# lighttransport/nanort

Measured on AMD Instinct MI355X. Metric: Mrays/s (primary + 1-bounce) at 1920x1080, 1M-tri mesh; BVH build ms, higher is better.
Workload: dtype f32; 1 GPU; C3: Plane(1000,500) = 1,000,000 triangles fp32; 1920x1080 objrender-camera primaries + 1 cosine bounce per hit (2073600 + 2055142 rays per GPU per step); parallelism=replicated BVH, interleaved image rows per GPU

## Files before the change

### nanort_amd/csrc/api.hip

```cpp
#include <hip/hip_runtime.h>
#include <stdarg.h>
#include <stdio.h>
#include <stdlib.h>
#include <string.h>
#include <ctype.h>
#include <math.h>
#include <cmath>

#include <algorithm>
#include <atomic>
#include <chrono>
#include <mutex>
#include <thread>
#include <string>
#include <vector>

#include "kernels.h"
#include "launch_plan.h"
#ifdef NRT_PROF
#include "../../include/nanort_hip_prof.h"
#endif

using namespace nrt;

// ... 43 lines not shown

  struct LaunchSlot {
    uint32_t *d_cursor = nullptr;
    unsigned parity = 0;
    DevBuf spill, spill_tmin;
    DevBuf cyl_hits, cyl_bits;
    hipEvent_t done = nullptr;
    hipEvent_t t0 = nullptr, t1 = nullptr;
    hipStream_t stream = nullptr;
    bool used = false;
    DoneRec *h_done = nullptr, *d_done = nullptr;
    DoneCount *d_count = nullptr;
    uint32_t seq = 0;
    bool rec_pending = false;
    bool last_has_rec = false;
    bool last_timed = false;
  };
  static constexpr int kSlots = 4;
  LaunchSlot slots[kSlots];
  unsigned next_victim = 0;
  std::mutex launch_mutex;
  std::mutex host_mutex;
  unsigned long long *d_counters = nullptr;
  DevBuf st_rays, st_hits, st_mask;
  hipStream_t copy_in = nullptr, copy_out = nullptr;
  hipEvent_t ev_in[2] = {nullptr, nullptr}, ev_tr[2] = {nullptr, nullptr}, ev_out[2] = {nullptr, nullptr};
  int host_pipeline = 1;
  DevBuf b_wave_clock;
  uint32_t wave_clock_waves = 0;

  int lds_stack = kLdsStackDefault;
  unsigned chunk = 128, chunk_tail_pct = 0, refill_min = 44, trav_min = 16, leaf_min = 32;
  int f64_row_fetch = 1;
  unsigned trav_min4 = 24;
  unsigned num_parts = 8;
  unsigned debug_flags = 0;
  int subtree_rows = 1;
  int morton = 0;
  unsigned static_pct = 16;
  unsigned static_bands = 8;
  unsigned static_slice_groups = 2;
  unsigned max_blocks_per_cu = 0;
  int wide = 1, wide_stack = 10;
  int wide4 = 1;
  int wide4_big_ok = 1;
  int order4 = 0;
  int leaf_compact = 1;
  int dyn_head = 1;
  int wide_scramble = 0;
  struct { int lds_entries; unsigned blocks_per_cu; } occupancy[4][kNumPrimKinds] = {};

  hipEvent_t ev_b0 = nullptr, ev_b1 = nullptr;
  hipEvent_t ev_build_state = nullptr;
  void *build_state = nullptr;
  int last_timed_slot = -1;
  int launch_timing = 0;
  bool have_build_time = false;
  float segment_ms = 0.f;
  const char *last_kernel = "";
};

static nrt_status fail(nrt_ctx *c, nrt_status st, const char *fmt, ...) {
  char buf[512];
  va_list ap;
  va_start(ap, fmt);
  vsnprintf(buf, sizeof(buf), fmt, ap);
// ... 99 lines not shown

struct TunableDesc {
  const char *name;
  long long lo, hi;
  long long (*get)(const nrt_ctx *);
  void (*set)(nrt_ctx *, long long);
};
#define NRT_TUNABLE(name_, lo_, hi_, field_, type_)                                                          \
  {name_, lo_, hi_, [](const nrt_ctx *c) -> long long { return (long long)c->field_; },                      \
   [](nrt_ctx *c, long long v) { c->field_ = (type_)v; }}
static const TunableDesc kTunables[] = {
    NRT_TUNABLE("refill_min", 1, 64, refill_min, unsigned),
    NRT_TUNABLE("trav_min", 1, 64, trav_min, unsigned),
    NRT_TUNABLE("trav_min4", 1, 64, trav_min4, unsigned),
    NRT_TUNABLE("f64_row_fetch", 0, 1, f64_row_fetch, int),
    NRT_TUNABLE("leaf_min", 1, 64, leaf_min, unsigned),
    NRT_TUNABLE("chunk_tail_pct", 0, 100, chunk_tail_pct, unsigned),
    NRT_TUNABLE("parts", 1, kMaxParts, num_parts, unsigned),
    NRT_TUNABLE("static_pct", 0, 100, static_pct, unsigned),
    NRT_TUNABLE("static_bands", 1, 64, static_bands, unsigned),
    NRT_TUNABLE("static_slice_groups", 1, 64, static_slice_groups, unsigned),
    NRT_TUNABLE("blocks_per_cu", 0, 8, max_blocks_per_cu, unsigned),
    NRT_TUNABLE("debug", 0, 0x7FFFFFFF, debug_flags, unsigned),
    NRT_TUNABLE("morton", 0, 1, morton, int),
    NRT_TUNABLE("cyl_split", 1, 64, cyl_split, int),
    NRT_TUNABLE("cyl_seg_radii", 1, 1024, cyl_seg_radii, int),
#ifdef NRT_PROF
    NRT_TUNABLE("subtree_rows", 0, 1, subtree_rows, int),
#endif
    NRT_TUNABLE("wide", 0, 1, wide, int),
    NRT_TUNABLE("wide4_big", 0, 2, wide4_big_ok, int),
    NRT_TUNABLE("wide4", 0, 1, wide4, int),
    NRT_TUNABLE("leaf_compact", 0, 1, leaf_compact, int),
    NRT_TUNABLE("dyn_head", 0, 1, dyn_head, int),
    NRT_TUNABLE("order4", 0, 1, order4, int),
    NRT_TUNABLE("launch_timing", 0, 1, launch_timing, int),
    NRT_TUNABLE("host_pipeline", 0, 1, host_pipeline, int),
    NRT_TUNABLE("wide_scramble", 0, 1, wide_scramble, int),
    {"chunk", 32, 1 << 20, [](const nrt_ctx *c) -> long long { return c->chunk; },
     [](nrt_ctx *c, long long v) { c->chunk = (unsigned)(v / 32) * 32u; }},
    {"lds_stack", 16, 32, [](const nrt_ctx *c) -> long long { return c->lds_stack; },
     [](nrt_ctx *c, long long v) { if (v == 16 || v == 24 || v == 32) c->lds_stack = (int)v; }},
    {"wide_stack", 8, 16, [](const nrt_ctx *c) -> long long { return c->wide_stack; },
     [](nrt_ctx *c, long long v) { if (v == 8 || v == 10 || v == 12 || v == 16) c->wide_stack = (int)v; }},
};
#undef NRT_TUNABLE

static const TunableDesc *tunable_find(const char *name) {
  if (!name) return nullptr;
  for (const TunableDesc &d : kTunables)
    if (!strcmp(d.name, name)) return &d;
  return nullptr;
}
static bool tunable_set(nrt_ctx *c, const char *name, long long v) {
  const TunableDesc *d = tunable_find(name);
  if (!d) return false;
  d->set(c, std::min(d->hi, std::max(d->lo, v)));
  memset(c->occupancy, 0, sizeof(c->occupancy));
  return true;
}

extern "C" {

const char *nrtVersion(void) { return "libnanort_hip 0.1 (gfx950, HIP)"; }

nrt_status nrtHostAlloc(size_t bytes, void **out) {
// ... 783 lines not shown
  const bool profiled = (w.dbg & (32u | 8192u)) != 0u;
  a.nodes = (const typename Wire<T>::Node *)c->d_nodes;
  a.tris = (const LeafTri<T> *)c->d_tris;
  a.spheres = (const LeafSphere<T> *)c->d_tris;
  a.centers = (const T *)c->d_verts;
  a.cylinders = (const LeafCylinder<T> *)c->d_tris;
  a.cyl_test_cap = c->cyl_test_cap;
  a.curves = (const LeafCurve *)c->d_tris;
  a.curve_subdiv = c->curve_subdiv;
  a.wide = (const WideNode<T> *)c->d_wide;
  a.wide4 = w.wide4() ? (const Wide4Node<T> *)c->d_wide4 : nullptr;
  a.packed_leaves = c->packed_leaves;
  a.wide4_big = (w.wide4() && w.wide4_big) ? 1u : 0u;
  a.wide_below_4g = (c->f64_row_fetch && (uint64_t)c->num_branch_records * sizeof(WideNode<T>) < (1ull << 32)) ? 1u : 0u;
  a.root_is_branch = c->root_is_branch;
  a.debug_flags = w.dbg;
  a.range0 = l.opt->prim_ids_range[0];
  a.range1 = l.opt->prim_ids_range[1];
  a.skip_prim = l.opt->skip_prim_id;
  a.cull_back_face = l.opt->cull_back_face ? 1u : 0u;
  a.any_hit = l.kind == Query::Occlusion ? 1u : 0u;
  a.plain_options = w.plain_options ? 1u : 0u;
  a.root_test = c->tree_nested ? 0u : 1u;
  a.order4 = (c->order4 && w.wide4() && c->prim_kind == kPrimTriangles && l.kind != Query::Occlusion && !profiled) ? 1u : 0u;
  a.leaf_items = (c->leaf_compact && w.wide4() && c->prim_kind == kPrimTriangles && c->max_leaf_count <= 4u && !profiled) ? 1u : 0u;
  a.dyn_head = c->dyn_head ? 1u : 0u;
  a.counters = c->d_counters;
  a.wave_clock = (w.dbg & 8192u) ? (unsigned long long *)c->b_wave_clock.p : nullptr;
  a.chunk = c->chunk;
  a.chunk_tail_pct = c->chunk_tail_pct;
  a.refill_min = c->refill_min;
  a.trav_min = w.wide4() ? c->trav_min4 : c->trav_min;
  a.leaf_min = c->leaf_min;
}

template <typename T>
static void fill_launch_args(const TraverseLaunch<T> &l, const nrt_ctx::LaunchSlot *slot, const GridPlan &g, const DistributionPlan &d,
                             uint32_t levels, TraverseArgs<T> &a) {
  a.spill = (uint32_t *)slot->spill.p;
  a.spill_tmin = (T *)slot->spill_tmin.p;
  a.spill_stride = g.grid * kTraverseBlock;
  a.spill_levels = levels;
  a.ray_cursor = slot->d_cursor + (size_t)slot->parity * kCursorStrideWords * kMaxParts;
  a.next_cursor = slot->d_cursor + (size_t)(slot->parity ^ 1u) * kCursorStrideWords * kMaxParts;
  a.num_parts = g.parts;
  a.blocks_per_part = g.blocks_per_part;
  a.static_per_wave = d.static_per_wave;
  a.static_bands = d.static_bands;
  a.band_len = d.band_len;
  a.band_static = d.band_static;
  a.dyn_per_band = d.dyn_per_band;
  a.dyn_banded = d.dyn_banded;
  a.tail_begin = d.tail_begin;
  a.dyn_total = d.dyn_total;
  a.dyn_per_part = d.dyn_per_part;
  a.rays = l.rays;
  a.hits = l.hits;
  a.mask = l.mask;
  if (l.kind == Query::Cylinders || l.kind == Query::Curves) {
    a.hits = (typename Wire<T>::Hit *)slot->cyl_hits.p;
    a.mask = (uint8_t *)slot->cyl_bits.p;
  }
  a.num_rays = (uint32_t)l.n;
  a.num_batches = 1u;
  a.batch_anyhit = 0u;
  for (int k = 0; k < kMaxBatches; k++) {
// ... 57 lines not shown
  if (timed) {
    HIPCHK(c, hipEventRecord(slot->t1, s));
    slot->last_timed = true;
    c->last_timed_slot = (int)(slot - c->slots);
  }
  if (!use_rec) HIPCHK(c, hipEventRecord(slot->done, s));
  return NRT_OK;
}

template <typename T>
static nrt_status traverse_device(nrt_ctx *c, TraverseLaunch<T> l) {
  if (!l.opt) l.opt = &kDefaultTrace;
  std::lock_guard<std::mutex> lock(c->launch_mutex);
  nrt_status st = validate_launch(c, l);
  if (st || l.n == 0) return st;
  HIPCHK(c, hipSetDevice(c->device));
  HIPCHK(c, refit_stream_wait(c, l.stream));
  nrt_ctx::LaunchSlot *slot = nullptr;
  if ((st = take_slot(c, l.stream, &slot))) return st;
  const WalkChoice w = choose_walk(c, l);
  const GridPlan g = size_grid<T>(c, w, l.n);
  const uint32_t total_threads = g.grid * kTraverseBlock, total_waves = g.grid * (kTraverseBlock / kWave);
  const DistributionPlan d = plan_distribution((uint32_t)l.n, total_waves, g.parts, c->static_pct, c->static_bands, c->static_slice_groups, c->chunk);
  const uint32_t levels = plan_spill_levels(c->tree_depth, w.wide4(), (uint32_t)w.lds_entries);
  if (levels) {
    if ((st = ensure(c, slot->spill, (size_t)levels * total_threads * sizeof(uint32_t)))) return st;
    if (w.wide() && (st = ensure(c, slot->spill_tmin, (size_t)levels * total_threads * sizeof(T)))) return st;
  }
  if (l.kind == Query::Cylinders || l.kind == Query::Curves) {
    if ((st = ensure(c, slot->cyl_hits, (size_t)l.n * sizeof(typename Wire<T>::Hit)))) return st;
    if ((st = ensure(c, slot->cyl_bits, (size_t)l.n))) return st;
  }
  if (w.dbg & 8192u) {
    if ((st = ensure(c, c->b_wave_clock, (size_t)total_waves * 3 * sizeof(unsigned long long)))) return st;
    c->wave_clock_waves = total_waves;
  }
  TraverseArgs<T> a;
  fill_walk_args(c, l, w, a);
  fill_launch_args(l, slot, g, d, levels, a);
  return enqueue_launch(c, l, w, slot, a, g.grid);
}

const uint64_t kStagedRays = 1ull << 26;

template <typename T, typename MakeLaunch>
static nrt_status staged_host_loop(nrt_ctx *c, const typename Wire<T>::Ray *rays, uint64_t n, uint64_t chunk, size_t rec_bytes, size_t flag_bytes,
                                   void *recs, void *flags, MakeLaunch make) {
  const size_t ray_bytes = sizeof(typename Wire<T>::Ray);
  for (uint64_t off = 0; off < n; off += chunk) {
    const uint64_t m = std::min(chunk, n - off);
    nrt_status st;
    if ((st = ensure(c, c->st_rays, m * ray_bytes)) || (rec_bytes && (st = ensure(c, c->st_hits, m * rec_bytes))) || (st = ensure(c, c->st_mask, m * flag_bytes)))
      return st;
    HIPCHK(c, hipMemcpyAsync(c->st_rays.p, rays + off, m * ray_bytes, hipMemcpyHostToDevice, c->stream));
    if ((st = traverse_device<T>(c, make(m)))) return st;
    if (recs) HIPCHK(c, hipMemcpyAsync((char *)recs + off * rec_bytes, c->st_hits.p, m * rec_bytes, hipMemcpyDeviceToHost, c->stream));
    if (flags) HIPCHK(c, hipMemcpyAsync((char *)flags + off * flag_bytes, c->st_mask.p, m * flag_bytes, hipMemcpyDeviceToHost, c->stream));
    HIPCHK(c, hipStreamSynchronize(c->stream));
  }
  return NRT_OK;
}
static bool is_pinned_host(const void *p) {
  hipPointerAttribute_t at;
  if (hipPointerGetAttributes(&at, p) != hipSuccess) {
    (void)hipGetLastError();
    return false;
  }
// ... 542 lines not shown
    nrt_ctx::LaunchSlot &sl = c->slots[c->last_timed_slot];
    if (sl.last_has_rec) {
      if (wait_record(sl) != hipSuccess) return -1.f;
      const unsigned long long b = sl.h_done->t_begin, e = sl.h_done->t_end;
      const hipStream_t s = sl.stream;
      lock.unlock();
      if (hipStreamSynchronize(s) != hipSuccess) return -1.f;
      return e >= b ? (float)((double)(e - b) * 1e-5) : -1.f;
    }
    if (!sl.last_timed) return -1.f;
    t0 = sl.t0;
    t1 = sl.t1;
  }
  if (hipEventSynchronize(t1) != hipSuccess) return -1.f;
  float ms = -1.f;
  if (hipEventElapsedTime(&ms, t0, t1) != hipSuccess) return -1.f;
  return ms;
}

const char *nrtLastKernelName(const nrt_ctx *c) { return c ? c->last_kernel : ""; }

#ifdef NRT_PROF
int nrtDebugCounters(nrt_ctx *c, unsigned long long *out, int cap) {
  if (!c || !out || cap < 16) return 1;
  if (hipStreamSynchronize(c->stream) != hipSuccess) return 1;
  if (hipDeviceSynchronize() != hipSuccess) return 1;
  return hipMemcpy(out, c->d_counters, 16 * sizeof(unsigned long long), hipMemcpyDeviceToHost) == hipSuccess ? 0 : 1;
}

long nrtDebugWaveClocks(nrt_ctx *c, unsigned long long *out, long cap) {
  if (!c || !out || !c->b_wave_clock.p) return -1;
  if (hipDeviceSynchronize() != hipSuccess) return -1;
  const long n = std::min<long>(cap, (long)c->wave_clock_waves);
  if (hipMemcpy(out, c->b_wave_clock.p, (size_t)n * 3 * sizeof(unsigned long long), hipMemcpyDeviceToHost) != hipSuccess) return -1;
  return (long)c->wave_clock_waves;
}

#endif

float nrtLastBuildMs(nrt_ctx *c) {
  if (!c || !c->have_build_time) return -1.f;
  return c->stats.build_secs * 1e3f;
}

}
```

### nanort_amd/csrc/common.h

```cpp
#pragma once

#include <hip/hip_runtime.h>
#include <stddef.h>
#include <stdint.h>
#include <stdlib.h>

#include "../../include/nanort_hip.h"
#include "walk_variant.h"

#ifdef NRT_ROCTX
#include <rocprofiler-sdk-roctx/roctx.h>
namespace nrt {
struct RoctxRange {
  explicit RoctxRange(const char *msg) { roctxRangePushA(msg); }
  ~RoctxRange() { roctxRangePop(); }
};
}
#define NRT_RANGE_CAT2(a, b) a##b
#define NRT_RANGE_CAT(a, b) NRT_RANGE_CAT2(a, b)
#define NRT_RANGE(msg) ::nrt::RoctxRange NRT_RANGE_CAT(nrt_range_, __LINE__)(msg)
#define NRT_RANGE_PUSH(msg) roctxRangePushA(msg)
#define NRT_RANGE_POP() roctxRangePop()
#else
#define NRT_RANGE(msg) do { } while (0)
// ... 94 lines not shown
};
static_assert(sizeof(LeafCurve) == 64, "LeafCurve");

template <typename T>
struct alignas(16) WideNode {
  T box0[6];
  T box1[6];
  uint32_t c0, c1;
  int32_t axis;
  uint32_t pad;
};
template <>
struct alignas(16) WideNode<double> {
  double mn[3][2];
  double mx[3][2];
  uint32_t c0, c1;
  int32_t axis;
  uint32_t pad;
};
static_assert(sizeof(WideNode<float>) == 64, "WideNode<float>");
static_assert(sizeof(WideNode<double>) == 112, "WideNode<double>");
template <typename T>
struct alignas(16) Wide4Node {
  T bmin[3][4];
  T bmax[3][4];
  uint32_t c[4];
  int32_t axis0, axis1, axis2;
  uint32_t pad;
};
static_assert(sizeof(Wide4Node<float>) == 128, "Wide4Node<float>");
static_assert(sizeof(Wide4Node<double>) == 224, "Wide4Node<double>");
constexpr uint32_t kWide4Empty = 0xFFFFFFFFu;
constexpr uint32_t kLeafBit = 0x80000000u;
constexpr uint32_t kPackedFirstBits = 27;
constexpr uint32_t kPackedFirstMask = (1u << kPackedFirstBits) - 1u;
constexpr uint32_t kPackedMaxCount = 16;

struct TreeViewF32 {
  const nrt_node_f32 *nodes;
  const uint32_t *indices;
  const void *wide;
  const void *wide4;
  const void *prims;
  uint32_t num_nodes, num_indices;
  uint32_t packed_leaves, root_is_branch, tree_nested, prim_kind, tree_depth;
  uint32_t max_leaf_count;
  uint64_t generation;
};

struct SceneInst {
  const void *wide;
  const void *wide4;
  const void *tris;
  const nrt_node_f32 *nodes;
  uint32_t packed_leaves, root_is_branch, tree_nested, pad;
  float inv_xform[4][4];
  float inv_xform33[4][4];
  float xform[4][4];
  float xbmin[3], xbmax[3];
  uint32_t id, pad2;
};
static_assert(sizeof(SceneInst) == 272, "SceneInst");
__device__ __forceinline__ bool scene_node_interval(const nrt_ray_f32 &r, const float xbmin[3], const float xbmax[3], float &t_min_out) {
  float tmin = r.min_t, tmax = r.max_t;
  float tn[3], tf[3];
#pragma unroll
// ... 134 lines not shown
  BatchPtrs batches[kMaxBatches];
  uint32_t range0, range1, skip_prim;
  uint32_t cull_back_face;
  uint32_t any_hit;
  uint32_t plain_options;
  uint32_t root_test;
  uint32_t leaf_items;
  uint32_t order4;
  uint32_t *spill;
  T *spill_tmin;
  uint32_t spill_stride;
  uint32_t spill_levels;
  uint32_t *ray_cursor;
  uint32_t *next_cursor;
  uint32_t num_parts;
  uint32_t static_per_wave;
  uint32_t static_bands;
  uint32_t band_len;
  uint32_t band_static;
  uint32_t dyn_per_band;
  uint32_t dyn_banded;
  uint32_t tail_begin;
  uint32_t dyn_total;
  uint32_t dyn_per_part;
  uint32_t blocks_per_part;
  uint32_t dyn_head;
  unsigned long long *counters;
  unsigned long long *wave_clock;
  uint32_t chunk;
  uint32_t chunk_tail_pct;
  uint32_t refill_min;
  uint32_t trav_min;
  uint32_t leaf_min;
  DoneRec *done_rec;
  DoneCount *done_count;
  uint32_t done_seq;
  uint32_t done_publish;
  const LeafCurve *curves;
  uint32_t curve_subdiv;
};

}
```

### nanort_amd/csrc/traverse.hip

```cpp
#include "kernels.h"
#include "traverse_dev.h"

#include <algorithm>

namespace nrt {

template <typename A>
static void launch_persistent(const void *kernel, unsigned grid, const A &args, hipStream_t s) {
  void *params[] = {(void *)&args};
  (void)hipLaunchKernel(kernel, dim3(grid), dim3(kTraverseBlock), params, 0, s);
}
static int resident_blocks(const void *kernel, int fallback) {
  int n = 0;
  if (hipOccupancyMaxActiveBlocksPerMultiprocessor(&n, kernel, kTraverseBlock, 0) != hipSuccess || n < 1) n = fallback;
  return n > 8 ? 8 : n;
}

template <typename T, bool COUNT, int STACK>
__global__ __launch_bounds__(kTraverseBlock) void k_traverse(const TraverseArgs<T> a) {
  __shared__ uint32_t s_stack[STACK][kTraverseBlock];

  typedef typename Wire<T>::Node Node;
  typedef typename Wire<T>::Ray Ray;
  typedef typename Wire<T>::Hit Hit;
// ... 712 lines not shown
  T tt_i = T(0), uu_i = T(0), vv_i = T(0);
  if (ok) {
    const T Az = sz * Akz, Bz = sz * Bkz, Cz = sz * Ckz;
    const T D = U * Az + V * Bz + W * Cz;
    const T rcp = T(1.0) / det;
    tt_i = D * rcp;
    uu_i = V * rcp;
    vv_i = W * rcp;
  }
  const unsigned long long okm_ = __ballot(ok);
  bool got_ = false;
  uint32_t win_ = 0;
  for (uint32_t k2_ = 0; k2_ < kmax_; k2_++) {
    const uint32_t src_ = (base_ + k2_) & 63u;
    const T ttk = __int_as_float(__builtin_amdgcn_ds_bpermute((int)(src_ << 2), __float_as_int(tt_i)));
    const bool okk = (k2_ < cnt) & (((okm_ >> src_) & 1ull) != 0ull);
    const bool acc = okk & !(ttk > L.hit_t) & !(ttk < L.min_t);
    L.hit_t = acc ? ttk : L.hit_t;
    win_ = acc ? src_ : win_;
    got_ = got_ | acc;
  }
  if (__ballot(got_) != 0ull) {
    const int wa_ = (int)(win_ << 2);
    const T uw = __int_as_float(__builtin_amdgcn_ds_bpermute(wa_, __float_as_int(uu_i)));
    const T vw = __int_as_float(__builtin_amdgcn_ds_bpermute(wa_, __float_as_int(vv_i)));
    const uint32_t pw = (uint32_t)__builtin_amdgcn_ds_bpermute(wa_, (int)prim_i);
    L.u = got_ ? uw : L.u;
    L.v = got_ ? vw : L.v;
    L.prim = got_ ? pw : L.prim;
  }
  return true;
}

template <typename T, int STACK, bool STATS, int KIND, bool PLAIN = false, bool CLOCK = false, int WIDTH = 2, int ORDER = 0>
__global__ __launch_bounds__(kTraverseBlock, (WIDTH == 4 && sizeof(T) == 4) ? NRT_W4_WAVES : 1) void k_traverse_wide(const TraverseArgs<T> a) {
  static_assert(WIDTH == 2 || WIDTH == 4, "one or two tree levels per step");
  static_assert(KIND != kPrimCurves || sizeof(T) == 4, "curves are fp32 only, as their example");
  static_assert(ORDER == 0 || (WIDTH == 4 && sizeof(T) == 4), "distance order / leaf items are variants of the fp32 two-level step");
  static_assert((ORDER & 2) == 0 || (KIND == kPrimTriangles && !STATS), "leaf items: triangle records, production instantiations");
  static_assert((ORDER & 4) == 0 || ((ORDER & 1) == 0 && KIND == kPrimTriangles && !STATS && !CLOCK), "records addressed by 64-bit offsets: the default walk of triangle trees");
  constexpr bool LEAFC = (ORDER & 2) != 0;
  constexpr bool BIG = (ORDER & 4) != 0;
  typedef typename std::conditional<BIG, uint64_t, uint32_t>::type RecOff;
  __shared__ uint32_t s_item_owner[LEAFC ? kTraverseBlock / kWave : 1][LEAFC ? kWave : 1];
  __shared__ uint32_t s_item_rec[LEAFC ? kTraverseBlock / kWave : 1][LEAFC ? kWave : 1];
  typedef StackEntry<T> SE;
  __shared__ typename SE::type s_stack[STACK][kTraverseBlock];

  typedef typename Wire<T>::Node Node;
  typedef typename Wire<T>::Ray Ray;
  typedef typename Wire<T>::Hit Hit;

  const unsigned tid = threadIdx.x;
  const unsigned lane = lane_id();
  const unsigned gslot = blockIdx.x * kTraverseBlock + tid;
  const bool cull = a.cull_back_face != 0;

  NRT_BATCH_TABLE_SETUP();
  Lane<T> L;
  uint32_t rid = kInvalid;
  uint32_t cur = 0;
  int state = W_IDLE;
  int sp = 0;
  const bool clocked = CLOCK && a.wave_clock != nullptr;
  unsigned long long clk_begin = 0ull, clk_dry = 0ull;
  if (clocked) clk_begin = __builtin_amdgcn_s_memrealtime();
  Claim ck;
  claim_init<T>(a, ck);
  if (blockIdx.x == 0 && threadIdx.x < kMaxParts)
    __hip_atomic_store(a.next_cursor + kCursorStrideWords * threadIdx.x, 0u, __ATOMIC_RELAXED, __HIP_MEMORY_SCOPE_AGENT);
  done_begin<T>(a);
  unsigned long long st_it1 = 0, st_act1 = 0, st_idle2 = 0, st_it2 = 0, st_act2 = 0, st_refills = 0, st_refilled = 0, st_entries2 = 0;
  uint32_t st_steps = 0, st_tris = 0;
  unsigned long long st_t_refill = 0, st_t_p1 = 0, st_t_p2 = 0, st_act2b = 0, st_stamp = 0;
  unsigned long long st_it1_s = 0, st_act1_s = 0, st_it2_s = 0, st_act2_s = 0;

#define NRT_WRITE_RESULT()                              \
  do {                                                  \
    const bool hit_ = L.hit_t < L.max_t;                \
    Hit h_;                                             \
    h_.u = hit_ ? L.u : T(0);                           \
    h_.v = hit_ ? L.v : T(0);                           \
    if (STATS && (a.debug_flags & 64u)) {               \
      h_.u = T(st_steps);                               \
      h_.v = T(st_tris);                                \
    }                                                   \
    h_.t = hit_ ? L.hit_t : L.max_t;                    \
    h_.prim_id = hit_ ? L.prim : kInvalid;              \
    Hit *hp_ = a.hits;                                  \
    uint8_t *mp_ = a.mask;                              \
    if (multi) {                                        \
      const BatchPtrs bp_ = s_tbl[batch_of<T>(a, rid)]; \
      hp_ = (Hit *)bp_.hits_v;                          \
      mp_ = bp_.mask_v;                                 \
    }                                                   \
    if (hp_) store_hit_nt<T>(hp_ + rid, h_);            \
    if (mp_) mp_[rid] = hit_ ? (KIND == kPrimCylinders ? (uint8_t)(1u | (L.cap << 1)) : (uint8_t)1) : (uint8_t)0; \
  } while (0)

// ... 38 lines not shown
            rp_ = (const Ray *)s_tbl[b_].rays_v;
            bq_ = (a.batch_anyhit >> b_) & 1u;
          }
          const Ray r = (a.debug_flags & 4u) ? rp_[rid] : load_ray_nt<T>(rp_ + rid);
          lane_init<T>(L, r);
          L.pk |= bq_ << 9;
          sp = 0;
          if (STATS) st_steps = st_tris = 0;
          if (a.root_is_branch && !a.root_test) {
            cur = 0u;
            state = W_TRAV;
          } else if (a.root_is_branch) {
            const Node root = a.nodes[0];
            cur = 0u;
            state = slab_test<T>(L, root.bmin, root.bmax) ? W_TRAV : W_POP;
          } else {
            const Node root = a.nodes[0];
            const bool root_hit = slab_test<T>(L, root.bmin, root.bmax);
            cur = a.packed_leaves ? (((root.data[0] - 1u) << kPackedFirstBits) | root.data[1]) : 0u;
            state = root_hit ? W_LEAF : W_POP;
          }
          if (a.debug_flags & 2u) state = W_POP;
        }
        if (STATS) {
          st_refills++;
          st_refilled += take;
        }
        ck.next += take;
        fresh = __ballot(state == W_IDLE);
      }
      idle = __ballot(state == W_IDLE);
    }
    if (clocked && ck.exhausted && clk_dry == 0ull) clk_dry = __builtin_amdgcn_s_memrealtime();
    if (idle == ~0ull) {
      if (ck.exhausted) break;
      continue;
    }

    if (STATS) {
      const unsigned long long now_ = __builtin_amdgcn_s_memtime();
      st_t_refill += now_ - st_stamp;
      st_stamp = now_;
    }
    unsigned n_wait_leaf = (unsigned)__builtin_popcountll(__ballot(state == W_LEAF));
    while (state == W_TRAV || state == W_POP) {
      if (STATS) {
        st_it1++;
        st_act1 += (unsigned)__builtin_popcountll(__ballot(true));
        if (!ck.exhausted) {
          st_it1_s++;
          st_act1_s += (unsigned)__builtin_popcountll(__ballot(true));
        }
      }
#pragma unroll
      for (int u_ = 0; u_ < ((WIDTH == 4 && sizeof(T) == 4 && !STATS) ? NRT_W4_P1_UNROLL : ((WIDTH == 2 && sizeof(T) == 8 && !STATS) ? NRT_W2_F64_P1_UNROLL : 1)); u_++) {
      if (state == W_POP) NRT_POP_ENTRY();
      if (state == W_TRAV) {
        if (STATS) st_steps++;
        if constexpr (WIDTH == 4) {
#if NRT_W4_PRESEL
          if constexpr (sizeof(T) == 4) {
            const char *wb_ = reinterpret_cast<const char *>(a.wide4);
            const RecOff rec_ = (RecOff)cur << 7;
            const Slab4<float> sl = slab4_presel<RecOff>(L, wb_, rec_);
            const Wide4Tail w = *reinterpret_cast<const Wide4Tail *>(wb_ + (size_t)rec_ + 96);
            if constexpr ((ORDER & 1) == 1)
// ... 16 lines not shown
#endif
#if NRT_W2_F64_PRESEL
          bool stepped_ = false;
          if constexpr (sizeof(T) == 8) {
            if (a.wide_below_4g) {
              const char *wb_ = reinterpret_cast<const char *>(a.wide);
              const uint32_t rec_ = cur * (uint32_t)sizeof(WideNode<double>);
              const SlabPair<double> sl = slab_pair_presel(L, wb_, rec_);
              const WideTail w = *reinterpret_cast<const WideTail *>(wb_ + (size_t)rec_ + 96);
              NRT_STEP_NODE_SL(sl, w);
              stepped_ = true;
            }
          }
          if (!stepped_)
#endif
          {
          const WideNode<T> w = a.wide[cur];
#ifdef NRT_PROBE_EXTRA_VALU
          {
            float f_ = __uint_as_float(cur);
            for (int x_ = 0; x_ < NRT_PROBE_EXTRA_VALU; x_++) asm volatile("v_fma_f32 %0, %0, %0, %0" : "+v"(f_));
            asm volatile("" :: "v"(f_));
          }
#endif
          NRT_STEP_NODE(w);
          }
#ifdef NRT_PROBE_EXTRA_LOADS
          asm volatile("" :: "v"(d0_));
#endif
        }
      }
      }
      n_wait_leaf += (unsigned)__builtin_popcountll(__ballot(state == W_LEAF));
      if ((unsigned)__builtin_popcountll(__ballot(state == W_TRAV || state == W_POP)) < a.trav_min &&
          (n_wait_leaf != 0u || !ck.exhausted))
        break;
    }

    if (STATS) {
      const unsigned long long now_ = __builtin_amdgcn_s_memtime();
      st_t_p1 += now_ - st_stamp;
      st_stamp = now_;
    }
    const unsigned n_leaf = (unsigned)__builtin_popcountll(__ballot(state == W_LEAF));
    const bool refill_due = !ck.exhausted && (unsigned)__builtin_popcountll(__ballot(state == W_IDLE)) >= a.refill_min;
    if (n_leaf != 0u && !(n_leaf < a.leaf_min && refill_due)) {
      uint32_t cnt = 0, first = 0;
      if (state == W_LEAF) {
        if (a.packed_leaves) {
          cnt = (cur >> kPackedFirstBits) + 1u;
          first = cur & kPackedFirstMask;
        } else {
          const Node *nd = a.nodes + cur;
          cnt = nd->data[0];
          first = nd->data[1];
        }
      }
      if (a.debug_flags & 1u) cnt = 0;
      if (STATS) {
        st_entries2++;
        st_idle2 += (unsigned)__builtin_popcountll(__ballot(state == W_IDLE));
      }
      bool items_done_ = false;
      if constexpr (LEAFC) {
        items_done_ = leaf_items_one_trip<PLAIN, uint32_t>(L, cnt, a.tris, first, lane, s_item_owner[tid / kWave], s_item_rec[tid / kWave], a.range0, a.range1,
                                                 a.skip_prim, cull);
      }
      if (items_done_) {
      } else if constexpr (KIND == kPrimTriangles && (WIDTH == 4 ? NRT_W4_TRI_UNROLL : NRT_W2_TRI_UNROLL) > 1) {
// ... 15 lines not shown
#pragma unroll
          for (uint32_t j = 0; j < U_; j++) {
            if (PLAIN)
              tri_test<T, true>(L, t_[j], i + j < cnt, 0u, 0u, 0u, false);
            else
              tri_test<T>(L, t_[j], i + j < cnt, a.range0, a.range1, a.skip_prim, cull);
          }
        }
      } else if constexpr (!STATS && KIND == kPrimSpheres && NRT_SPHERE_UNROLL > 1) {
        for (uint32_t i = 0; __ballot(i < cnt) != 0ull; i += NRT_SPHERE_UNROLL) {
          LeafSphere<T> s_[NRT_SPHERE_UNROLL];
#pragma unroll
          for (uint32_t j = 0; j < NRT_SPHERE_UNROLL; j++) s_[j] = a.spheres[first + (i + j < cnt ? i + j : 0u)];
#pragma unroll
          for (uint32_t j = 0; j < NRT_SPHERE_UNROLL; j++) sphere_test<T>(L, s_[j], i + j < cnt, a.range0, a.range1);
        }
      } else
      for (uint32_t i = 0; __ballot(i < cnt) != 0ull; i++) {
        if (STATS) {
          st_it2++;
          st_act2 += (unsigned)__builtin_popcountll(__ballot(i < cnt));
          if (i < cnt) st_tris++;
        }
        NRT_TEST_PRIM(first + (i < cnt ? i : 0u), i < cnt);
      }
      if (a.any_hit | a.batch_anyhit) sp = (state == W_LEAF && L.hit_t < L.max_t && (a.any_hit != 0u || (L.pk & 512u) != 0u)) ? 0 : sp;
      state = (state == W_LEAF) ? W_POP : state;
    }
    if (STATS) st_t_p2 += __builtin_amdgcn_s_memtime() - st_stamp;
  }
  if (rid != kInvalid) NRT_WRITE_RESULT();
#undef NRT_WRITE_RESULT
#undef NRT_TEST_PRIM
  done_end<T>(a, lane);
  if (clocked && lane == 0u) {
    unsigned long long *rec = a.wave_clock + 3ull * (size_t)(gslot / kWave);
    const unsigned long long clk_end = __builtin_amdgcn_s_memrealtime();
    rec[0] = clk_begin;
    rec[1] = clk_dry == 0ull ? clk_end : clk_dry;
    rec[2] = clk_end;
  }
  if (STATS && lane == 0) {
    atomicAdd(&a.counters[0], st_it1);
    atomicAdd(&a.counters[1], st_act1);
    atomicAdd(&a.counters[2], st_idle2);
    atomicAdd(&a.counters[3], st_it2);
    atomicAdd(&a.counters[4], st_act2);
    atomicAdd(&a.counters[5], st_refills);
    atomicAdd(&a.counters[6], st_refilled);
    atomicAdd(&a.counters[7], st_entries2);
    atomicAdd(&a.counters[8], st_t_refill);
    atomicAdd(&a.counters[9], st_t_p1);
    atomicAdd(&a.counters[10], st_t_p2);
    atomicAdd(&a.counters[11], st_act2b);
    atomicAdd(&a.counters[12], st_it1_s);
    atomicAdd(&a.counters[13], st_act1_s);
    atomicAdd(&a.counters[14], st_it2_s);
    atomicAdd(&a.counters[15], st_act2_s);
  }
}

template <typename R>
__device__ __forceinline__ R load_global_record(const R *p) {
  R r;
  if constexpr (sizeof(R) % 16 == 0 && alignof(R) >= 16) {
    typedef uint32_t u4g __attribute__((ext_vector_type(4)));
    const u4g __attribute__((address_space(1))) *g = (const u4g __attribute__((address_space(1))) *)p;
    u4g *d = reinterpret_cast<u4g *>(&r);
#pragma unroll
    for (unsigned q = 0; q < sizeof(R) / 16; q++) d[q] = g[q];
  } else {
    static_assert(sizeof(R) % 4 == 0, "whole words");
    const uint32_t __attribute__((address_space(1))) *g = (const uint32_t __attribute__((address_space(1))) *)p;
// ... 981 lines not shown
```

Measured before the change: 6814 Mrays/s.

## Spread tail rays across lane quads for cooperative wide4 traversal

Once the ray pool is exhausted and a wave has at most tail_quad live rays, their state is compacted with ds_bpermute so each ray is owned by a 4-lane quad. The quad then processes one ray together: each lane tests one child box of a wide4 node, stack pushes are ordered through DPP quad reductions, and leaf triangles are split four ways with a quad-wide closest-hit vote. This targets the long low-occupancy tail of divergent waves, at the cost of a large extra code path that can add register pressure and shuffle overhead. It also adds wave-clock stamps for the 16/8/4-live points and grows the wave clock record to six words.

```diff
diff --git a/nanort_amd/csrc/api.hip b/nanort_amd/csrc/api.hip
--- a/nanort_amd/csrc/api.hip
+++ b/nanort_amd/csrc/api.hip
@@ -99,6 +99,7 @@
   int lds_stack = kLdsStackDefault;
   unsigned chunk = 128, chunk_tail_pct = 0, refill_min = 44, trav_min = 16, leaf_min = 32;
   int f64_row_fetch = 1;
+  unsigned tail_quad = 4;
   unsigned trav_min4 = 24;
   unsigned num_parts = 8;
   unsigned debug_flags = 0;
@@ -264,6 +265,7 @@
     NRT_TUNABLE("wide4_big", 0, 2, wide4_big_ok, int),
     NRT_TUNABLE("wide4", 0, 1, wide4, int),
     NRT_TUNABLE("leaf_compact", 0, 1, leaf_compact, int),
+    NRT_TUNABLE("tail_quad", 0, 16, tail_quad, unsigned),
     NRT_TUNABLE("dyn_head", 0, 1, dyn_head, int),
     NRT_TUNABLE("order4", 0, 1, order4, int),
     NRT_TUNABLE("launch_timing", 0, 1, launch_timing, int),
@@ -1113,6 +1115,7 @@
   a.refill_min = c->refill_min;
   a.trav_min = w.wide4() ? c->trav_min4 : c->trav_min;
   a.leaf_min = c->leaf_min;
+  a.tail_lanes = c->tail_quad;
 }
 
 template <typename T>
@@ -1236,7 +1239,7 @@
     if ((st = ensure(c, slot->cyl_bits, (size_t)l.n))) return st;
   }
   if (w.dbg & 8192u) {
-    if ((st = ensure(c, c->b_wave_clock, (size_t)total_waves * 3 * sizeof(unsigned long long)))) return st;
+    if ((st = ensure(c, c->b_wave_clock, (size_t)total_waves * kWaveClockWords * sizeof(unsigned long long)))) return st;
     c->wave_clock_waves = total_waves;
   }
   TraverseArgs<T> a;
@@ -1845,7 +1848,7 @@
   if (!c || !out || !c->b_wave_clock.p) return -1;
   if (hipDeviceSynchronize() != hipSuccess) return -1;
   const long n = std::min<long>(cap, (long)c->wave_clock_waves);
-  if (hipMemcpy(out, c->b_wave_clock.p, (size_t)n * 3 * sizeof(unsigned long long), hipMemcpyDeviceToHost) != hipSuccess) return -1;
+  if (hipMemcpy(out, c->b_wave_clock.p, (size_t)n * kWaveClockWords * sizeof(unsigned long long), hipMemcpyDeviceToHost) != hipSuccess) return -1;
   return (long)c->wave_clock_waves;
 }
 
diff --git a/nanort_amd/csrc/common.h b/nanort_amd/csrc/common.h
--- a/nanort_amd/csrc/common.h
+++ b/nanort_amd/csrc/common.h
@@ -150,6 +150,7 @@
 static_assert(sizeof(Wide4Node<double>) == 224, "Wide4Node<double>");
 constexpr uint32_t kWide4Empty = 0xFFFFFFFFu;
 constexpr uint32_t kLeafBit = 0x80000000u;
+constexpr int kWaveClockWords = 6;
 constexpr uint32_t kPackedFirstBits = 27;
 constexpr uint32_t kPackedFirstMask = (1u << kPackedFirstBits) - 1u;
 constexpr uint32_t kPackedMaxCount = 16;
@@ -350,6 +351,7 @@
   uint32_t refill_min;
   uint32_t trav_min;
   uint32_t leaf_min;
+  uint32_t tail_lanes;
   DoneRec *done_rec;
   DoneCount *done_count;
   uint32_t done_seq;
diff --git a/nanort_amd/csrc/traverse.hip b/nanort_amd/csrc/traverse.hip
--- a/nanort_amd/csrc/traverse.hip
+++ b/nanort_amd/csrc/traverse.hip
@@ -768,6 +768,16 @@
   return true;
 }
 
+__device__ __forceinline__ uint32_t quad_or(uint32_t x) {
+  x |= (uint32_t)__builtin_amdgcn_update_dpp(0, (int)x, 0xB1, 0xF, 0xF, true);
+  x |= (uint32_t)__builtin_amdgcn_update_dpp(0, (int)x, 0x4E, 0xF, 0xF, true);
+  return x;
+}
+template <int K>
+__device__ __forceinline__ float quad_bcast(float v) {
+  return __int_as_float(__builtin_amdgcn_update_dpp(0, __float_as_int(v), K * 0x55, 0xF, 0xF, true));
+}
+
 template <typename T, int STACK, bool STATS, int KIND, bool PLAIN = false, bool CLOCK = false, int WIDTH = 2, int ORDER = 0>
 __global__ __launch_bounds__(kTraverseBlock, (WIDTH == 4 && sizeof(T) == 4) ? NRT_W4_WAVES : 1) void k_traverse_wide(const TraverseArgs<T> a) {
   static_assert(WIDTH == 2 || WIDTH == 4, "one or two tree levels per step");
@@ -778,6 +788,7 @@
   constexpr bool LEAFC = (ORDER & 2) != 0;
   constexpr bool BIG = (ORDER & 4) != 0;
   typedef typename std::conditional<BIG, uint64_t, uint32_t>::type RecOff;
+  constexpr bool QUAD = WIDTH == 4 && sizeof(T) == 4 && KIND == kPrimTriangles && !STATS && (ORDER & 1) == 0 && !BIG;
   __shared__ uint32_t s_item_owner[LEAFC ? kTraverseBlock / kWave : 1][LEAFC ? kWave : 1];
   __shared__ uint32_t s_item_rec[LEAFC ? kTraverseBlock / kWave : 1][LEAFC ? kWave : 1];
   typedef StackEntry<T> SE;
@@ -800,7 +811,20 @@
   int sp = 0;
   const bool clocked = CLOCK && a.wave_clock != nullptr;
   unsigned long long clk_begin = 0ull, clk_dry = 0ull;
+  unsigned long long clk_l16 = 0ull, clk_l8 = 0ull, clk_l4 = 0ull;
   if (clocked) clk_begin = __builtin_amdgcn_s_memrealtime();
+#define NRT_TAIL_N (a.tail_lanes < 16u ? a.tail_lanes : 16u)
+#define NRT_CLOCK_LIVE(live_)                                                  \
+  do {                                                                         \
+    if constexpr (CLOCK) {                                                     \
+      if (clocked && ck.exhausted && clk_l4 == 0ull && (live_) <= 16u) {       \
+        const unsigned long long now_ = __builtin_amdgcn_s_memrealtime();      \
+        if (clk_l16 == 0ull) clk_l16 = now_;                                   \
+        if (clk_l8 == 0ull && (live_) <= 8u) clk_l8 = now_;                    \
+        if ((live_) <= 4u) clk_l4 = now_;                                      \
+      }                                                                        \
+    }                                                                          \
+  } while (0)
   Claim ck;
   claim_init<T>(a, ck);
   if (blockIdx.x == 0 && threadIdx.x < kMaxParts)
@@ -905,6 +929,213 @@
       idle = __ballot(state == W_IDLE);
     }
     if (clocked && ck.exhausted && clk_dry == 0ull) clk_dry = __builtin_amdgcn_s_memrealtime();
+    NRT_CLOCK_LIVE(64u - (unsigned)__builtin_popcountll(idle));
+    if constexpr (QUAD) {
+      const unsigned live_n_ = 64u - (unsigned)__builtin_popcountll(idle);
+      if (ck.exhausted && live_n_ != 0u && live_n_ <= NRT_TAIL_N) {
+        if (state == W_IDLE && rid != kInvalid) NRT_WRITE_RESULT();
+        const unsigned q_ = lane >> 2, j_ = lane & 3u;
+        uint32_t src_ = 0u;
+        {
+          unsigned k_ = 0u;
+          for (unsigned long long m_ = ~idle; m_ != 0ull; m_ &= m_ - 1ull, k_++) src_ = (q_ == k_) ? (uint32_t)__builtin_ctzll(m_) : src_;
+        }
+        const bool has_ = q_ < live_n_;
+        const int sa_ = (int)(src_ << 2);
+#define NRT_QMOVE_F(x_) x_ = __int_as_float(__builtin_amdgcn_ds_bpermute(sa_, __float_as_int(x_)))
+#define NRT_QMOVE_U(x_) x_ = (uint32_t)__builtin_amdgcn_ds_bpermute(sa_, (int)(x_))
+        NRT_QMOVE_F(L.org0);
+        NRT_QMOVE_F(L.org1);
+        NRT_QMOVE_F(L.org2);
+        NRT_QMOVE_F(L.inv0);
+        NRT_QMOVE_F(L.inv1);
+        NRT_QMOVE_F(L.inv2);
+        NRT_QMOVE_F(L.min_t);
+        NRT_QMOVE_F(L.max_t);
+        NRT_QMOVE_F(L.hit_t);
+        NRT_QMOVE_F(L.Sx);
+        NRT_QMOVE_F(L.Sy);
+        NRT_QMOVE_F(L.Sz);
+        NRT_QMOVE_F(L.u);
+        NRT_QMOVE_F(L.v);
+        NRT_QMOVE_U(L.pk);
+        NRT_QMOVE_U(L.prim);
+        NRT_QMOVE_U(rid);
+        NRT_QMOVE_U(cur);
+        state = __builtin_amdgcn_ds_bpermute(sa_, state);
+        sp = __builtin_amdgcn_ds_bpermute(sa_, sp);
+#undef NRT_QMOVE_F
+#undef NRT_QMOVE_U
+        L.so0 = (L.pk & 1u) ? 48u : 0u;
+        L.so1 = (L.pk & 2u) ? 48u : 0u;
+        L.so2 = (L.pk & 4u) ? 48u : 0u;
+        state = has_ ? state : W_IDLE;
+        rid = has_ ? rid : kInvalid;
+        sp = has_ ? sp : 0;
+        const unsigned otid_ = (tid & ~63u) | src_;
+        const unsigned ogslot_ = blockIdx.x * kTraverseBlock + otid_;
+        bool owner_ = j_ == 0u;
+        const char *wb_ = reinterpret_cast<const char *>(a.wide4);
+        for (;;) {
+          const unsigned long long liveq_ = __ballot(state != W_IDLE);
+          NRT_CLOCK_LIVE((unsigned)__builtin_popcountll(liveq_) >> 2);
+          if (liveq_ == 0ull) break;
+          if (state == W_POP) {
+            int s1_ = sp - 1;
+            s1_ = s1_ < 0 ? 0 : s1_;
+            const int sl_ = s1_ > STACK - 1 ? STACK - 1 : s1_;
+            typename SE::type e_ = s_stack[sl_][otid_];
+            if (s1_ >= STACK) {
+              const size_t o_ = (size_t)(s1_ - STACK) * a.spill_stride + ogslot_;
+              e_ = SE::make(a.spill[o_], a.spill_tmin[o_]);
+            }
+            const bool fin_ = (sp == 0);
+            const bool enter_ = !fin_ & (SE::tmin(e_) <= L.hit_t);
+            const uint32_t ref_ = SE::ref(e_);
+            sp = s1_;
+            cur = enter_ ? (ref_ & ~kLeafBit) : cur;
+            state = fin_ ? W_IDLE : (enter_ ? ((ref_ & kLeafBit) ? W_LEAF : W_TRAV) : W_POP);
+          }
+          if (state == W_TRAV) {
+            const uint32_t rec0_ = cur << 7, rec_ = rec0_ + 4u * j_, rec48_ = rec_ + 48u;
+            const float lo0 = *reinterpret_cast<const float *>(wb_ + (size_t)(rec_ + L.so0));
+            const float hi0 = *reinterpret_cast<const float *>(wb_ + (size_t)(rec48_ - L.so0));
+            const float lo1 = *reinterpret_cast<const float *>(wb_ + (size_t)(rec_ + L.so1) + 16);
+            const float hi1 = *reinterpret_cast<const float *>(wb_ + (size_t)(rec48_ - L.so1) + 16);
+            const float lo2 = *reinterpret_cast<const float *>(wb_ + (size_t)(rec_ + L.so2) + 32);
+            const float hi2 = *reinterpret_cast<const float *>(wb_ + (size_t)(rec48_ - L.so2) + 32);
+            const uint32_t c_ = *reinterpret_cast<const uint32_t *>(wb_ + (size_t)rec_ + 96);
+            const int ax0_ = *reinterpret_cast<const int32_t *>(wb_ + (size_t)rec0_ + 112);
+            const int axh_ = *reinterpret_cast<const int32_t *>(wb_ + (size_t)(rec0_ + 4u * (j_ >> 1)) + 116);
+            const float mm = Const<float>::maxmult();
+            float tmin = L.min_t, tmax = L.hit_t;
+            {
+              const float t0 = (lo0 - L.org0) * L.inv0;
+              const float t1 = ((hi0 - L.org0) * L.inv0) * mm;
+              tmin = Const<float>::fmax(t0, tmin);
+              tmax = Const<float>::fmin(t1, tmax);
+            }
+            {
+              const float t0 = (lo1 - L.org1) * L.inv1;
+              const float t1 = ((hi1 - L.org1) * L.inv1) * mm;
+              tmin = Const<float>::fmax(t0, tmin);
+              tmax = Const<float>::fmin(t1, tmax);
+            }
+            {
+              const float t0 = (lo2 - L.org2) * L.inv2;
+              const float t1 = ((hi2 - L.org2) * L.inv2) * mm;
+              tmin = Const<float>::fmax(t0, tmin);
+              tmax = Const<float>::fmin(t1, tmax);
+            }
+            const bool h_ = (tmin <= tmax) & (((j_ & 1u) == 0u) | (c_ != kWide4Empty));
+            const uint32_t s0_ = (uint32_t)L.sign(ax0_), sh_ = (uint32_t)L.sign(axh_);
+            const uint32_t rank_ = ((((j_ >> 1) ^ s0_) & 1u) << 1) | ((j_ ^ sh_) & 1u);
+            const uint32_t m_ = quad_or(h_ ? (1u << rank_) : 0u);
+            const uint32_t n_ = (uint32_t)__builtin_popcount(m_);
+            const uint32_t pos_ = (uint32_t)__builtin_popcount(m_ & ((1u << rank_) - 1u));
+            if (h_ && pos_ != 0u) {
+              const int at_ = sp + (int)(n_ - 1u - pos_);
+              if (at_ < STACK) {
+                s_stack[at_][otid_] = SE::make(c_, tmin);
+              } else {
+                const size_t o_ = (size_t)(at_ - STACK) * a.spill_stride + ogslot_;
+                a.spill[o_] = c_;
+                a.spill_tmin[o_] = tmin;
+              }
+            }
+            __builtin_amdgcn_fence(__ATOMIC_RELEASE, "wavefront");
+            sp += n_ != 0u ? (int)(n_ - 1u) : 0;
+            const uint32_t next_ = quad_or((h_ && pos_ == 0u) ? c_ : 0u);
+            cur = n_ != 0u ? (next_ & ~kLeafBit) : cur;
+            state = n_ != 0u ? ((next_ & kLeafBit) ? W_LEAF : W_TRAV) : W_POP;
+          }
+          if (__ballot(state == W_LEAF) != 0ull) {
+            uint32_t cnt = 0, first = 0;
+            if (state == W_LEAF) {
+              if (a.packed_leaves) {
+                cnt = (cur >> kPackedFirstBits) + 1u;
+                first = cur & kPackedFirstMask;
+              } else {
+                const Node *nd = a.nodes + cur;
+                cnt = nd->data[0];
+                first = nd->data[1];
+              }
+            }
+            if (a.debug_flags & 1u) cnt = 0;
+            for (uint32_t i = 0; __ballot(i < cnt) != 0ull; i += 4u) {
+              const bool act_ = i + j_ < cnt;
+              const LeafTri<T> tri = a.tris[first + (act_ ? i + j_ : 0u)];
+              const uint32_t prim_i = tri.prim_id;
+              bool ok = PLAIN ? act_ : (act_ & (prim_i >= a.range0) & (prim_i < a.range1) & (prim_i != a.skip_prim));
+              const bool cull_i = PLAIN ? false : cull;
+              const T A0 = tri.p0[0] - L.org0, A1 = tri.p0[1] - L.org1, A2 = tri.p0[2] - L.org2;
+              const T B0 = tri.p1[0] - L.org0, B1 = tri.p1[1] - L.org1, B2 = tri.p1[2] - L.org2;
+              const T C0 = tri.p2[0] - L.org0, C1 = tri.p2[1] - L.org1, C2 = tri.p2[2] - L.org2;
+              const T Akz = sel3(A0, A1, A2, L.kz()), Bkz = sel3(B0, B1, B2, L.kz()), Ckz = sel3(C0, C1, C2, L.kz());
+              const T Ax = sel3(A0, A1, A2, L.kx()) - L.Sx * Akz;
+              const T Ay = sel3(A0, A1, A2, L.ky()) - L.Sy * Akz;
+              const T Bx = sel3(B0, B1, B2, L.kx()) - L.Sx * Bkz;
+              const T By = sel3(B0, B1, B2, L.ky()) - L.Sy * Bkz;
+              const T Cx = sel3(C0, C1, C2, L.kx()) - L.Sx * Ckz;
+              const T Cy = sel3(C0, C1, C2, L.ky()) - L.Sy * Ckz;
+              T U = Cx * By - Cy * Bx;
+              T V = Ax * Cy - Ay * Cx;
+              T W = Bx * Ay - By * Ax;
+              if (ok && (U == T(0) || V == T(0) || W == T(0))) {
+                const double CxBy = double(Cx) * double(By), CyBx = double(Cy) * double(Bx);
+                const double AxCy = double(Ax) * double(Cy), AyCx = double(Ay) * double(Cx);
+                const double BxAy = double(Bx) * double(Ay), ByAx = double(By) * double(Ax);
+                U = T(CxBy - CyBx);
+                V = T(AxCy - AyCx);
+                W = T(BxAy - ByAx);
+              }
+              const bool neg = (U < T(0)) | (V < T(0)) | (W < T(0));
+              const bool pos = (U > T(0)) | (V > T(0)) | (W > T(0));
+              ok = ok & !(neg & (cull_i | pos));
+              const T det = U + V + W;
+              ok = ok & !(det == T(0));
+              T tt_i = T(0), uu_i = T(0), vv_i = T(0);
+              if (ok) {
+                const T Az = L.Sz * Akz, Bz = L.Sz * Bkz, Cz = L.Sz * Ckz;
+                const T D = U * Az + V * Bz + W * Cz;
+                const T rcp = T(1.0) / det;
+                tt_i = D * rcp;
+                uu_i = V * rcp;
+                vv_i = W * rcp;
+              }
+              const uint32_t okm_ = quad_or(ok ? (1u << j_) : 0u);
+              if (__ballot(okm_ != 0u) != 0ull) {
+                bool got_ = false;
+                uint32_t win_ = 0u;
+#define NRT_QUAD_ACCEPT(K_)                                                                                                    \
+                do {                                                                                                           \
+                  const T ttk_ = quad_bcast<K_>(tt_i);                                                                         \
+                  const bool acc_ = ((okm_ >> K_) & 1u) != 0u && !(ttk_ > L.hit_t) && !(ttk_ < L.min_t);  \
+                  L.hit_t = acc_ ? ttk_ : L.hit_t;                                                                             \
+                  win_ = acc_ ? (uint32_t)K_ : win_;                                                                           \
+                  got_ = got_ | acc_;                                                                                          \
+                } while (0)
+                NRT_QUAD_ACCEPT(0);
+                NRT_QUAD_ACCEPT(1);
+                NRT_QUAD_ACCEPT(2);
+                NRT_QUAD_ACCEPT(3);
+#undef NRT_QUAD_ACCEPT
+                const bool me_ = got_ & (win_ == j_);
+                owner_ = got_ ? me_ : owner_;
+                L.u = me_ ? uu_i : L.u;
+                L.v = me_ ? vv_i : L.v;
+                L.prim = me_ ? prim_i : L.prim;
+              }
+            }
+            if (a.any_hit | a.batch_anyhit) sp = (state == W_LEAF && L.hit_t < L.max_t && (a.any_hit != 0u || (L.pk & 512u) != 0u)) ? 0 : sp;
+            state = (state == W_LEAF) ? W_POP : state;
+          }
+        }
+        if (owner_ && rid != kInvalid) NRT_WRITE_RESULT();
+        rid = kInvalid;
+        break;
+      }
+    }
     if (idle == ~0ull) {
       if (ck.exhausted) break;
       continue;
@@ -987,9 +1218,15 @@
       }
       }
       n_wait_leaf += (unsigned)__builtin_popcountll(__ballot(state == W_LEAF));
-      if ((unsigned)__builtin_popcountll(__ballot(state == W_TRAV || state == W_POP)) < a.trav_min &&
-          (n_wait_leaf != 0u || !ck.exhausted))
-        break;
+      const unsigned n_walk_ = (unsigned)__builtin_popcountll(__ballot(state == W_TRAV || state == W_POP));
+      NRT_CLOCK_LIVE(n_walk_ + n_wait_leaf);
+      if (n_walk_ < a.trav_min && (n_wait_leaf != 0u || !ck.exhausted)) break;
+      if constexpr (QUAD) {
+        if (ck.exhausted && n_walk_ + n_wait_leaf <= NRT_TAIL_N) break;
+      }
+    }
+    if constexpr (QUAD) {
+      if (ck.exhausted && (unsigned)__builtin_popcountll(__ballot(state != W_IDLE)) <= NRT_TAIL_N) continue;
     }
 
     if (STATS) {
@@ -1071,13 +1308,18 @@
   if (rid != kInvalid) NRT_WRITE_RESULT();
 #undef NRT_WRITE_RESULT
 #undef NRT_TEST_PRIM
+#undef NRT_CLOCK_LIVE
+#undef NRT_TAIL_N
   done_end<T>(a, lane);
   if (clocked && lane == 0u) {
-    unsigned long long *rec = a.wave_clock + 3ull * (size_t)(gslot / kWave);
+    unsigned long long *rec = a.wave_clock + (size_t)kWaveClockWords * (size_t)(gslot / kWave);
     const unsigned long long clk_end = __builtin_amdgcn_s_memrealtime();
     rec[0] = clk_begin;
     rec[1] = clk_dry == 0ull ? clk_end : clk_dry;
     rec[2] = clk_end;
+    rec[3] = clk_l16 == 0ull ? clk_end : clk_l16;
+    rec[4] = clk_l8 == 0ull ? clk_end : clk_l8;
+    rec[5] = clk_l4 == 0ull ? clk_end : clk_l4;
   }
   if (STATS && lane == 0) {
     atomicAdd(&a.counters[0], st_it1);
```

After: 6971 Mrays/s (median of 6 runs). 1.02x the previous value.
